# AnamarijaKic/bioinfo1

Hardware: AMD Instinct MI355X
Metric: GCUPS (DP cell updates/s) at 1/2/4/8 GPUs; bit-exact score+CIGAR (higher is better)
Workload: dtype int32 semantics; packed int16 arithmetic where range-proven (fits_int16), else int32; 1 GPU; config 2: 10000 uniform 1000x1000 pairs per GPU, local, scoring 1,-1,-1, CIGAR on; pairs_per_gpu=10000, qlen=1000, tlen=1000, mode=local, cigar=True, cells_per_gpu=10000000000, cells_total=10000000000, parallelism=pairs range-split over 1 GPU(s)

## Files before the change

bioinfo1_amd/align.py:

```python
from __future__ import annotations

import ctypes as C
import enum
import os
from dataclasses import dataclass

import numpy as np

HERE = os.path.dirname(os.path.abspath(__file__))
LIB_PATH = os.path.join(HERE, "libteam_alignment.so")

TA_OK, TA_ERR_BAD_TYPE, TA_ERR_CIGAR, TA_ERR_ARG, TA_ERR_DEVICE, TA_ERR_CAPACITY, TA_ERR_RANGE, TA_ERR_UNSERVED = range(8)
TA_PLAN_INT32_ONLY, TA_PLAN_NO_FLEX, TA_PLAN_UNFUSED, TA_PLAN_WALK1, TA_PLAN_WALK2 = 1, 2, 4, 8, 16
TA_PLAN_SERIAL_PASSES, TA_PLAN_PASS_MAJOR, TA_PLAN_NO_BLK, TA_PLAN_NO_CK, TA_PLAN_CK = 32, 64, 128, 256, 512
TA_PLAN_NO_FLEX_CK = 1024


class AlignmentType(enum.IntEnum):

    global_ = 0
    local = 1
    semiGlobal = 2


# ... 27 lines not shown
    L.ta_cigar_slot_bytes.argtypes = [C.c_uint32, C.c_uint32]
    L.ta_align_batch.argtypes = [C.c_void_p, C.c_uint32, C.c_void_p, u64p, u32p, C.c_void_p, u64p, u32p, C.c_int,
                                 C.c_int, C.c_int, C.c_int, C.c_int, i32p, u32p, C.c_void_p, C.c_uint64, u64p, u32p]
    L.ta_align_batch_flags.argtypes = L.ta_align_batch.argtypes + [C.c_uint32]
    L.ta_context_release.argtypes = [C.c_void_p]
    L.ta_context_release.restype = None
    L.ta_context_held_bytes.argtypes = [C.c_void_p]
    L.ta_context_held_bytes.restype = C.c_uint64
    L.ta_set_default_device.argtypes = [C.c_int]
    L.ta_set_thread_device.argtypes = [C.c_int]
    L.ta_plan_create.argtypes = [C.c_void_p, C.c_uint32, u32p, u32p, C.c_int, C.c_int, C.c_int, C.c_int, C.c_int,
                                 C.c_uint64, C.c_uint32, C.POINTER(C.c_void_p)]
    L.ta_plan_destroy.argtypes = [C.c_void_p]
    L.ta_plan_destroy.restype = None
    for f in ("ta_plan_cigar_slots_bytes", "ta_plan_workspace_bytes"):
        getattr(L, f).restype = C.c_uint64
        getattr(L, f).argtypes = [C.c_void_p]
    L.ta_plan_chunks.restype = C.c_uint32
    L.ta_plan_chunks.argtypes = [C.c_void_p]
    L.ta_plan_dual_pairs.restype = C.c_uint32
    L.ta_plan_dual_pairs.argtypes = [C.c_void_p]
    L.ta_plan_flex_pairs.restype = C.c_uint32
    L.ta_plan_flex_pairs.argtypes = [C.c_void_p]
    L.ta_plan_fused.argtypes = [C.c_void_p]
    L.ta_plan_walk.argtypes = [C.c_void_p]
    L.ta_plan_pair_chunks.argtypes = [C.c_void_p, u32p]
    L.ta_affine_plan_pair_chunks.argtypes = [C.c_void_p, u32p]
    L.ta_plan_execute.argtypes = [C.c_void_p, C.c_void_p, C.c_void_p]
    L.ta_plan_check.argtypes = [C.c_void_p]
    L.ta_compact_cigars.argtypes = [C.c_void_p, C.c_uint32, C.c_void_p, C.c_void_p, C.c_void_p, C.c_void_p,
                                    C.c_void_p, C.c_void_p]
    L.ta_plan_execute_fill.argtypes = [C.c_void_p, C.c_void_p, C.c_void_p, C.c_uint32]
    L.ta_plan_execute_traceback.argtypes = [C.c_void_p, C.c_void_p, C.c_void_p, C.c_uint32]
    L.ta_align_batch_affine.argtypes = [C.c_void_p, C.c_uint32, C.c_void_p, u64p, u32p, C.c_void_p, u64p, u32p,
                                        C.c_int, C.c_int, C.c_int, C.c_int, C.c_int, C.c_int, i32p, u32p, C.c_void_p,
                                        C.c_uint64, u64p, u32p]
    L.ta_affine_plan_create.argtypes = [C.c_void_p, C.c_uint32, u32p, u32p, C.c_int, C.c_int, C.c_int, C.c_int,
                                        C.c_int, C.c_int, C.c_uint64, C.c_uint32, C.POINTER(C.c_void_p)]
    L.ta_affine_plan_destroy.argtypes = [C.c_void_p]
    L.ta_affine_plan_destroy.restype = None
    for f in ("ta_affine_plan_cigar_slots_bytes", "ta_affine_plan_workspace_bytes"):
        getattr(L, f).restype = C.c_uint64
        getattr(L, f).argtypes = [C.c_void_p]
    L.ta_affine_plan_chunks.restype = C.c_uint32
    L.ta_affine_plan_chunks.argtypes = [C.c_void_p]
    L.ta_affine_plan_dual_pairs.restype = C.c_uint32
    L.ta_affine_plan_dual_pairs.argtypes = [C.c_void_p]
    L.ta_affine_plan_execute.argtypes = [C.c_void_p, C.c_void_p, C.c_void_p]
    L.ta_affine_plan_execute_fill.argtypes = [C.c_void_p, C.c_void_p, C.c_void_p, C.c_uint32]
    L.ta_affine_plan_execute_traceback.argtypes = [C.c_void_p, C.c_void_p, C.c_void_p, C.c_uint32]
    L.ta_affine_plan_check.argtypes = [C.c_void_p]
    L.ta_align_batch_banded.argtypes = [C.c_void_p, C.c_uint32, C.c_void_p, u64p, u32p, C.c_void_p, u64p, u32p, u32p,
                                        C.c_int, C.c_int, C.c_int, C.c_int, C.c_int, i32p, u32p, C.c_void_p,
                                        C.c_uint64, u64p, u32p]
    L.ta_banded_plan_create.argtypes = [C.c_void_p, C.c_uint32, u32p, u32p, u32p, C.c_int, C.c_int, C.c_int, C.c_int,
                                        C.c_int, C.c_uint64, C.c_uint32, C.POINTER(C.c_void_p)]
    L.ta_banded_plan_destroy.argtypes = [C.c_void_p]
    L.ta_banded_plan_destroy.restype = None
    for f in ("ta_banded_plan_cigar_slots_bytes", "ta_banded_plan_workspace_bytes", "ta_banded_plan_band_cells",
              "ta_banded_plan_swept_cells"):
        getattr(L, f).restype = C.c_uint64
        getattr(L, f).argtypes = [C.c_void_p]
    L.ta_banded_plan_chunks.restype = C.c_uint32
    L.ta_banded_plan_chunks.argtypes = [C.c_void_p]
    L.ta_banded_plan_pair_chunks.argtypes = [C.c_void_p, u32p]
    L.ta_banded_plan_execute.argtypes = [C.c_void_p, C.c_void_p, C.c_void_p]
    L.ta_banded_plan_execute_fill.argtypes = [C.c_void_p, C.c_void_p, C.c_void_p, C.c_uint32]
    L.ta_banded_plan_execute_traceback.argtypes = [C.c_void_p, C.c_void_p, C.c_void_p, C.c_uint32]
    L.ta_banded_plan_check.argtypes = [C.c_void_p]
    L.ta_banded_plan_annotate.argtypes = [C.c_void_p, C.c_void_p, C.c_void_p, C.c_void_p]
    L.ta_plan_annotate.argtypes = [C.c_void_p, C.c_void_p, C.c_void_p, C.c_void_p]
    L.ta_affine_plan_annotate.argtypes = [C.c_void_p, C.c_void_p, C.c_void_p, C.c_void_p]
    L.ta_server_create.argtypes = [C.c_int, C.c_int, C.c_uint32, C.POINTER(C.c_void_p)]
    L.ta_server_destroy.argtypes = [C.c_void_p]
    L.ta_server_destroy.restype = None
    L.ta_server_fits.argtypes = [C.c_void_p, C.c_uint32, C.c_uint32, C.c_int, C.c_int, C.c_int]
    L.ta_server_running.argtypes = [C.c_void_p]
    L.ta_server_last_times.argtypes = [C.c_void_p, C.c_uint32, C.POINTER(C.c_double)]
    L.ta_server_align.argtypes = [C.c_void_p, C.c_char_p, C.c_uint32, C.c_char_p, C.c_uint32, C.c_int, C.c_int,
                                  C.c_int, C.c_int, C.POINTER(C.c_int32), C.POINTER(C.c_uint32), C.c_void_p,
                                  C.c_uint64, C.POINTER(C.c_uint32)]
    _lib = L
    return L


ABI_SYMBOLS = [
    "ta_status_string", "ta_last_error", "ta_context_create", "ta_context_destroy", "ta_context_release",
    "ta_context_held_bytes", "ta_set_default_device", "ta_set_thread_device", "ta_current_device", "ta_device_count",
    "ta_cigar_slot_bytes", "ta_align_batch", "ta_align_batch_flags", "ta_plan_create", "ta_plan_destroy", "ta_plan_cigar_slots_bytes",
    "ta_plan_workspace_bytes", "ta_plan_chunks", "ta_plan_dual_pairs", "ta_plan_flex_pairs", "ta_plan_fused", "ta_plan_walk",
    "ta_plan_execute", "ta_plan_check", "ta_plan_execute_fill", "ta_plan_pair_chunks", "ta_affine_plan_pair_chunks", "ta_plan_execute_traceback", "ta_compact_cigars",
    "ta_affine_plan_create", "ta_affine_plan_destroy", "ta_affine_plan_cigar_slots_bytes",
    "ta_affine_plan_workspace_bytes", "ta_affine_plan_chunks", "ta_affine_plan_dual_pairs", "ta_affine_plan_execute", "ta_affine_plan_execute_fill",
    "ta_affine_plan_execute_traceback", "ta_affine_plan_check", "ta_align_batch_affine",
    "ta_server_create", "ta_server_destroy", "ta_server_fits", "ta_server_align", "ta_server_running",
    "ta_server_last_times", "ta_server_pause", "ta_server_resume",
    "ta_plan_annotate", "ta_affine_plan_annotate",
]
BANDED_ABI_SYMBOLS = [
    "ta_banded_plan_create", "ta_banded_plan_destroy", "ta_banded_plan_cigar_slots_bytes",
    "ta_banded_plan_workspace_bytes", "ta_banded_plan_chunks", "ta_banded_plan_pair_chunks",
    "ta_banded_plan_band_cells", "ta_banded_plan_swept_cells", "ta_banded_plan_execute",
    "ta_banded_plan_execute_fill", "ta_banded_plan_execute_traceback", "ta_banded_plan_check",
    "ta_banded_plan_annotate", "ta_align_batch_banded",
]
ABI_SYMBOLS += BANDED_ABI_SYMBOLS
TEAM_ALIGN_SYMBOL = ("_ZN4team5AlignEPKcjS1_jNS_13AlignmentTypeEiiiPNSt7__cxx1112basic_stringIcSt11char_traitsIcESaIcEEEPj")


def _check_type(type) -> int:
    t = int(type)
    if t not in (0, 1, 2):
        raise ValueError("Unknown AlignmentType provided.")
    return t


def _raise(status: int, ctx=None):
    L = lib()
    msg = L.ta_status_string(status).decode()
    if status in (TA_ERR_BAD_TYPE, TA_ERR_CIGAR, TA_ERR_RANGE):
        raise ValueError(msg)
    detail = L.ta_last_error(ctx).decode() if ctx else ""
    raise DeviceError(f"{msg}: {detail}" if detail else msg)


def _p(a, ct):
    return a.ctypes.data_as(C.POINTER(ct))


def _band_array(band, n_pairs: int) -> np.ndarray:
# ... 415 lines not shown
        idx = torch.as_tensor(np.asarray(indices, np.int64), device=self.dev)
        sc = self.score[idx].cpu().numpy()
        tb = self.target_begin[idx].cpu().numpy().view(np.uint32)
        if not self.want_cigar:
            return BatchResult(sc, tb, None, None, None)
        start = self.cigar_start[idx].cpu().numpy()
        ln = self.cigar_len[idx].cpu().numpy().view(np.uint32)
        parts, offs, o = [], np.zeros(len(ln), np.uint64), 0
        for k in range(len(ln)):
            parts.append(self.slots[int(start[k]):int(start[k]) + int(ln[k])].cpu().numpy())
            offs[k] = o
            o += int(ln[k])
        arena = np.concatenate(parts) if parts else np.zeros(1, np.uint8)
        return BatchResult(sc, tb, offs, ln, arena)

    def results(self) -> BatchResult:
        self.check()
        return _results(self)

    def close(self):
        if getattr(self, "_h", None):
            self._fn("ta_plan_destroy")(self._h)
            self._h = None

    def __del__(self):
        try:
            self.close()
        except Exception:
            pass


class DevicePipeline:

    def __init__(self, device: int, batch, type, match, mismatch, gap, want_cigar=True, depth: int = 2,
                 workspace_budget: int = 0, gap_open=None, flags: int = 0, inputs=None, first=None):
        import torch

        self.torch = torch
        self.dev = torch.device("cuda", device)
        self.aligners, self.plans = [], []
        for k in range(depth):
            if k == 0 and first is not None:
                self.plans.append(first)
                continue
            al = Aligner(device)
            self.aligners.append(al)
            shared = inputs if not self.plans else (self.plans[0].qbytes, self.plans[0].qoff,
                                                    self.plans[0].tbytes, self.plans[0].toff)
            self.plans.append(DevicePlan(al, batch, type, match, mismatch, gap, want_cigar,
                                         workspace_budget=workspace_budget, gap_open=gap_open, flags=flags,
                                         inputs=shared))
        self.fill = torch.cuda.Stream(self.dev)
        self.walk = torch.cuda.Stream(self.dev, priority=-1)
        for st in (self.fill, self.walk):
            st.wait_stream(torch.cuda.current_stream(self.dev))
        self.walked = [torch.cuda.Event() for _ in range(depth)]
        self.done = [torch.cuda.Event() for _ in range(depth)]
        self.used = [False] * depth
        self.k = 0
        self.last = None

    @property
    def chunks(self):
        return self.plans[0].chunks

    def step(self, inputs=None, ready=None):
        torch = self.torch
        cur = torch.cuda.current_stream(self.dev)
        depth = len(self.plans)
        if self.last is not None:
            self.done[self.last].record(cur)
        i = self.k % depth
        self.k += 1
        plan = self.plans[i]
        if self.used[i]:
            self.fill.wait_event(self.done[i])
        if inputs is not None:
            plan.set_inputs(inputs)
            if ready is not None:
                self.fill.wait_event(ready)
        for c in range(plan.chunks):
            with torch.cuda.stream(self.fill):
                plan.run_fill(c)
            with torch.cuda.stream(self.walk):
                plan.run_traceback(c)
        self.walked[i].record(self.walk)
        cur.wait_event(self.walked[i])
        self.used[i] = True
        self.last = i
        return plan

    def check(self):
        for p in self.plans:
            p.check()

    def close(self):
        for p in self.plans:
            p.close()
        for al in self.aligners:
            al.close()


class HostBatchRunner:

    def __init__(self, aligner: Aligner, batch, type, match, mismatch, gap, want_cigar=True):
        import torch

        self.t = _check_type(type)
        self.sc = (match, mismatch, gap)
        self.want_cigar = bool(want_cigar)
        self.aligner = aligner
        self.P = P = batch.n_pairs

        def pinned(a):
            a = np.ascontiguousarray(a)
            t = torch.empty(max(a.nbytes, 1), dtype=torch.uint8, pin_memory=True)
            v = t.numpy()[: a.nbytes].view(a.dtype)
            v[...] = a.reshape(-1)
            return t, v

        self._keep = []
        for name, a in (("qb", batch.qbytes if batch.qbytes.size else np.zeros(1, np.uint8)), ("qoff", batch.qoff),
                        ("qlen", batch.qlen), ("tb", batch.tbytes if batch.tbytes.size else np.zeros(1, np.uint8)),
                        ("toff", batch.toff), ("tlen", batch.tlen), ("score", np.zeros(P, np.int32)),
                        ("tbeg", np.zeros(P, np.uint32)), ("coff", np.zeros(P, np.uint64)),
                        ("clen", np.zeros(P, np.uint32))):
            t, v = pinned(a)
            self._keep.append(t)
            setattr(self, name, v)
# ... 130 lines not shown
```

bioinfo1_amd/csrc/ta_affine.hip:

```cpp
#include <hip/hip_runtime.h>
#include <rocprofiler-sdk-roctx/roctx.h>

#include <algorithm>
#include <cstdlib>
#include <cstring>
#include <numeric>
#include <string>
#include <vector>

#include "../../include/team_align_c.h"
#include "ta_context.h"
#include "ta_device.h"
#include "ta_host_batch.h"
#include "ta_planner.h"
#include "ta_packed.h"

namespace ta {
namespace {

constexpr int kNeg = -(1 << 29);

struct AffArgs {
    const uint32_t* order;
    uint32_t begin, count;
// ... 1222 lines not shown
    AffOffs o = aff_layout(pl->h, L);
    const uint64_t upload = L.bytes;
    aff_layout_scratch(pl->h, L, o);
    std::vector<uint8_t> host(upload);
    aff_pack(pl->h, o, host.data());
    hipError_t e = hipMalloc(&pl->own_block, std::max<uint64_t>(L.bytes, 256));
    if (e == hipSuccess) e = hipMemcpy(pl->own_block, host.data(), upload, hipMemcpyHostToDevice);
    if (e != hipSuccess) {
        ta_affine_plan_destroy(pl);
        return fail(ctx, TA_ERR_DEVICE, std::string("ta_affine_plan_create: ") + hipGetErrorString(e));
    }
    aff_bind(pl, static_cast<uint8_t*>(pl->own_block), o);
    *out = pl;
    return TA_OK;
}

uint64_t ta_affine_plan_cigar_slots_bytes(const ta_affine_plan* pl) { return pl ? pl->h.slots_bytes : 0; }

int ta_affine_plan_check(ta_affine_plan* pl) {
    if (!pl) return TA_ERR_ARG;
    if (pl->h.duals.empty() && pl->h.single_tasks.empty()) return TA_OK;
    uint32_t err = 0;
    TA_HIP(pl->ctx, hipSetDevice(pl->ctx->device));
    TA_HIP(pl->ctx, hipMemcpy(&err, pl->d_err, 4, hipMemcpyDeviceToHost));
    if (!err) return TA_OK;
    TA_HIP(pl->ctx, hipMemset(pl->d_err, 0, 4));
    return fail(pl->ctx, TA_ERR_DEVICE,
                "affine fill: a pass hand-off poll timed out; results of this plan are invalid");
}
uint64_t ta_affine_plan_workspace_bytes(const ta_affine_plan* pl) {
    return pl ? pl->h.ws_ptr_entries * sizeof(uint2) + pl->h.ws_bnd_entries * sizeof(int2) : 0;
}
uint32_t ta_affine_plan_chunks(const ta_affine_plan* pl) { return pl ? (uint32_t)pl->h.chunks.size() : 0; }
uint32_t ta_affine_plan_dual_pairs(const ta_affine_plan* pl) { return pl ? (uint32_t)pl->h.duals.size() : 0; }

int ta_affine_plan_pair_chunks(const ta_affine_plan* pl, uint32_t* chunk_of_pair) {
    if (!pl || !chunk_of_pair) return TA_ERR_ARG;
    for (uint32_t c = 0; c < (uint32_t)pl->h.chunks.size(); ++c) {
        const auto& ch = pl->h.chunks[c];
        for (uint32_t k = ch.begin; k < ch.begin + ch.count; ++k) chunk_of_pair[pl->h.order[k]] = c;
    }
    return TA_OK;
}

int ta_affine_plan_execute(ta_affine_plan* pl, const ta_device_io* io, void* stream) {
    if (int r = affine_check_io(pl, io)) return r;
    std::lock_guard<std::mutex> lock(pl->ctx->mu);
    return affine_exec(pl, io, (hipStream_t)stream, UINT32_MAX, true, true);
}

int ta_affine_plan_annotate(ta_affine_plan* pl, const ta_device_io* io, const ta_annotate_io* out, void* stream) {
    if (!pl || !io || !out) return TA_ERR_ARG;
    ta_context* ctx = pl->ctx;
    if (!pl->h.want_cigar) return fail(ctx, TA_ERR_ARG, "annotate: the plan has no CIGARs");
    if (out->eqx_slots && (!out->eqx_start || !out->eqx_len)) return fail(ctx, TA_ERR_ARG, "annotate: eqx_slots without eqx_start / eqx_len");
    if (int r = affine_check_io(pl, io)) return r;
    if (!pl->h.n_pairs) return TA_OK;
    std::lock_guard<std::mutex> lock(ctx->mu);
    TA_HIP(ctx, hipSetDevice(ctx->device));
    ta::AnnotateArgs a{pl->h.n_pairs, pl->h.type, pl->d_qlen, pl->d_tlen, pl->d_goal_i, pl->d_goal_j, pl->d_slot_off,
                       reinterpret_cast<const uint8_t*>(io->query_bytes), io->query_off,
                       reinterpret_cast<const uint8_t*>(io->target_bytes), io->target_off, io->cigar_slots,
                       io->cigar_start, io->cigar_len, out->info, out->eqx_slots, out->eqx_start, out->eqx_len};
    TA_HIP(ctx, ta::launch_annotate(a, (hipStream_t)stream));
    return TA_OK;
}
// ... 40 lines not shown
```

bioinfo1_amd/csrc/ta_api.hip:

```cpp
#include <hip/hip_runtime.h>
#include <rocprofiler-sdk-roctx/roctx.h>

#include <algorithm>
#include <cstdio>
#include <cstdlib>
#include <cstring>
#include <mutex>
#include <string>
#include <vector>

#include "../../include/team_align_c.h"
#include "ta_context.h"
#include "ta_host_batch.h"
#include "ta_internal.h"
#include "ta_planner.h"

using ta_host::fail;

struct ta_plan {
    ta_context* ctx = nullptr;
    ta::Plan h;
    void* own_block = nullptr;
    uint32_t *d_qlen = nullptr, *d_tlen = nullptr, *d_order = nullptr, *d_singles = nullptr, *d_duals = nullptr,
             *d_flexes = nullptr;
    uint64_t *d_ptr_off = nullptr, *d_bnd_off = nullptr, *d_slot_off = nullptr;
    uint32_t *d_goal_i = nullptr, *d_goal_j = nullptr;
    uint32_t* d_fb = nullptr;
    uint32_t *d_flex_task_off = nullptr, *d_tickets = nullptr, *d_err = nullptr, *d_flex_tasks = nullptr;
    void* d_pout = nullptr;
    void* d_dpout = nullptr;
    uint32_t* d_stask_off = nullptr;
    uint64_t* d_stasks = nullptr;
    void* d_spout = nullptr;
    uint8_t* d_pflag = nullptr;
};

namespace {

bool valid_type(int t) { return t == TA_GLOBAL || t == TA_LOCAL || t == TA_SEMI_GLOBAL; }

struct PlanOffs {
    uint64_t qlen, tlen, order, singles, duals, flexes, task_off, tasks, stask_off, stasks, ptr_off, bnd_off, slot_off,
        err, tickets;
    uint64_t goal_i, goal_j, fb, pout, dpout, spout, pflag;
};

uint64_t dual_pout_bytes(const ta::Plan& h) {
// ... 182 lines not shown
                if (ch.fcount) {
                    if (int r = ta_host::lazy_stream(ctx, ctx->aux2)) return r;
                    TA_HIP(ctx, hipEventRecord(ctx->ev_fork, s));
                    TA_HIP(ctx, hipStreamWaitEvent(ctx->aux2, ctx->ev_fork, 0));
                    TA_HIP(ctx, ta::launch_dual(h.type, h.want_cigar, d, ctx->aux2));
                    TA_HIP(ctx, hipEventRecord(ctx->ev_join2, ctx->aux2));
                } else {
                    TA_HIP(ctx, ta::launch_dual(h.type, h.want_cigar, d, s));
                }
            }
            if (ch.fcount) {
                ta::FillArgs d = a;
                d.order = pl->d_flexes;
                d.begin = ch.fbegin;
                d.count = ch.fcount;
                d.fb_list = fb_list;
                d.fb_count = fb_count;
                d.task_off = pl->d_flex_task_off;
                d.tasks = pl->d_flex_tasks;
                d.ticket = pl->d_tickets + c;
                d.n_tasks = h.flex_task_off[ch.fbegin + ch.fcount] - h.flex_task_off[ch.fbegin];
                d.epoch = ++ctx->epoch & 0x3FFFFFFu;
                d.err = pl->d_err;
                d.pout = pl->d_pout;
                TA_HIP(ctx, hipMemsetAsync(d.ticket, 0, 4, s));
                TA_HIP(ctx, ta::launch_flex(h.type, h.want_cigar, d, s));
            }
            if (ch.dcount && ch.fcount) TA_HIP(ctx, hipStreamWaitEvent(s, ctx->ev_join2, 0));
            ta::FillArgs f = a;
            f.order = fb_list;
            f.begin = 0;
            f.count = 2 * (ch.dcount + ch.fcount);
            f.count_dev = fb_count;
            TA_HIP(ctx, ta::launch_fill(h.type, h.want_cigar, h.wide, f, s));
        }
        if (ch.scount && (ch.dcount || ch.fcount)) {
            TA_HIP(ctx, hipEventRecord(ctx->ev_join, ctx->aux));
            TA_HIP(ctx, hipStreamWaitEvent(s, ctx->ev_join, 0));
        }
        roctxRangePop();
    }
    if (trace && h.want_cigar && !h.fused) {
        roctxRangePushA("ta traceback");
        ta::TraceArgs t{};
        t.order = pl->d_order;
        t.begin = ch.begin;
        t.count = ch.count;
        t.qlen = pl->d_qlen;
        t.tlen = pl->d_tlen;
        t.ptrs = d_ptrs;
        t.ptr_off = pl->d_ptr_off;
        t.goal_i = pl->d_goal_i;
        t.goal_j = pl->d_goal_j;
        t.slots = io->cigar_slots;
        t.slot_off = pl->d_slot_off;
        t.cigar_start = io->cigar_start;
        t.cigar_len = io->cigar_len;
        t.score = io->score;
        t.qbytes = reinterpret_cast<const uint8_t*>(io->query_bytes);
        t.qoff = io->query_off;
        t.tbytes = reinterpret_cast<const uint8_t*>(io->target_bytes);
        t.toff = io->target_off;
        t.match = h.match;
        t.mismatch = h.mismatch;
        t.gap = h.gap;
        t.blk = h.blk ? (h.ck ? 2u : 1u) : 0u;
// ... 147 lines not shown
    if (!out) return TA_ERR_ARG;
    *out = nullptr;
    if (int r = check_args(ctx, n_pairs, qlen, tlen, type)) return r;
    TA_HIP(ctx, hipSetDevice(ctx->device));
    auto* pl = new ta_plan();
    pl->ctx = ctx;
    ta::build_plan(pl->h, n_pairs, qlen, tlen, type, match, mismatch, gap, want_cigar != 0,
                   budget ? budget : ta_host::default_budget(ctx), flags, 4 * ctx->cu_count);
    ta::BlockLayout L;
    PlanOffs o = layout_uploaded(pl->h, L);
    const uint64_t upload = L.bytes;
    layout_scratch(pl->h, L, o);
    std::vector<uint8_t> host(upload);
    pack(pl->h, o, host.data());
    hipError_t e = hipMalloc(&pl->own_block, std::max<uint64_t>(L.bytes, 256));
    if (e == hipSuccess) e = hipMemcpy(pl->own_block, host.data(), upload, hipMemcpyHostToDevice);
    if (e != hipSuccess) {
        ta_plan_destroy(pl);
        return fail(ctx, TA_ERR_DEVICE, std::string("ta_plan_create: ") + hipGetErrorString(e));
    }
    bind(pl, static_cast<uint8_t*>(pl->own_block), o);
    *out = pl;
    return TA_OK;
}

uint64_t ta_plan_cigar_slots_bytes(const ta_plan* pl) { return pl ? pl->h.slots_bytes : 0; }
uint64_t ta_plan_workspace_bytes(const ta_plan* pl) {
    if (!pl) return 0;
    const ta::Plan& h = pl->h;
    const uint64_t runs = (h.walk_group == 64 && h.want_cigar) ? 4 * (h.slots_bytes + 4) : 0;
    return (h.ws_ptr_dwords + h.ws_bnd_words) * 4ull + runs;
}
uint32_t ta_plan_chunks(const ta_plan* pl) { return pl ? (uint32_t)pl->h.chunks.size() : 0; }
uint32_t ta_plan_dual_pairs(const ta_plan* pl) { return pl ? pl->h.n_dual_pairs : 0; }
uint32_t ta_plan_flex_pairs(const ta_plan* pl) { return pl ? (uint32_t)pl->h.flexes.size() : 0; }
int ta_plan_fused(const ta_plan* pl) { return pl && pl->h.fused ? 1 : 0; }

int ta_plan_walk(const ta_plan* pl) {
    if (!pl) return -1;
    return pl->h.walk_group | (pl->h.blk ? 0x100 : 0) | (pl->h.ck ? 0x200 : 0);
}

int ta_plan_pair_chunks(const ta_plan* pl, uint32_t* chunk_of_pair) {
    if (!pl || !chunk_of_pair) return TA_ERR_ARG;
    for (uint32_t c = 0; c < (uint32_t)pl->h.chunks.size(); ++c) {
        const auto& ch = pl->h.chunks[c];
        for (uint32_t k = ch.begin; k < ch.begin + ch.count; ++k) chunk_of_pair[pl->h.order[k]] = c;
    }
    return TA_OK;
}

int ta_plan_execute(ta_plan* pl, const ta_device_io* io, void* stream) {
    if (int r = check_io(pl, io)) return r;
    std::lock_guard<std::mutex> lock(pl->ctx->mu);
    return exec(pl, io, (hipStream_t)stream, UINT32_MAX, true, true);
}

int ta_plan_execute_fill(ta_plan* pl, const ta_device_io* io, void* stream, uint32_t chunk) {
    if (int r = check_io(pl, io)) return r;
    if (chunk >= pl->h.chunks.size()) return pl->h.n_pairs ? TA_ERR_ARG : TA_OK;
    std::lock_guard<std::mutex> lock(pl->ctx->mu);
    return exec(pl, io, (hipStream_t)stream, chunk, true, false);
}

int ta_plan_execute_traceback(ta_plan* pl, const ta_device_io* io, void* stream, uint32_t chunk) {
    if (int r = check_io(pl, io)) return r;
// ... 75 lines not shown
```

bioinfo1_amd/csrc/ta_internal.h:

```cpp
#pragma once

#include <hip/hip_runtime.h>
#include <stdint.h>

#include "../../include/team_align_c.h"
#include "ta_layout.h"

namespace ta {

enum Code : uint32_t { kCodeM = 0, kCodeI = 1, kCodeD = 2, kCodeStop = 3 };
constexpr int kDPlane = 16;

struct FillArgs {
    const uint32_t* order;
    uint32_t begin, count;
    const uint8_t* qbytes;
    const uint64_t* qoff;
    const uint32_t* qlen;
    const uint8_t* tbytes;
    const uint64_t* toff;
    const uint32_t* tlen;
    int match, mismatch, gap;
    uint32_t* ptrs;
    const uint64_t* ptr_off;
    int32_t* bnd;
    const uint64_t* bnd_off;
    int32_t* score;
    uint32_t* target_begin;
    uint32_t* goal_i;
    uint32_t* goal_j;
    int fused;
    char* slots;
    const uint64_t* slot_off;
    uint64_t* cigar_start;
    uint32_t* cigar_len;
    uint32_t* fb_list;
    uint32_t* fb_count;
    const uint32_t* count_dev;
    const uint32_t* task_off;
    const uint32_t* tasks;
    uint32_t* ticket;
    uint32_t n_tasks;
    uint32_t epoch;
    uint32_t* err;
    void* pout;
    const uint64_t* tasks64;
    uint32_t end_aligned;
    uint32_t blk;
    uint8_t* pflag;
};

constexpr uint32_t kErrPassPoll = 1u;
constexpr uint32_t kErrWalkCap = 2u;
__host__ __device__ inline uint64_t band_runs_off(uint64_t slot_off) { return (slot_off + 3u) & ~(uint64_t)3u; }

struct TraceArgs {
    const uint32_t* order;
    uint32_t begin, count;
    const uint32_t* qlen;
    const uint32_t* tlen;
    const uint32_t* ptrs;
    const uint64_t* ptr_off;
    const uint32_t* goal_i;
    const uint32_t* goal_j;
    char* slots;
    const uint64_t* slot_off;
    uint64_t* cigar_start;
    uint32_t* cigar_len;
    const int32_t* score;
    const uint8_t* qbytes;
    const uint64_t* qoff;
// ... 97 lines not shown
```

bioinfo1_amd/csrc/ta_kernels.hip:

```cpp
#include <algorithm>
#include <cstdlib>

#include "ta_device.h"
#include "ta_walk2.h"
#include "ta_walk_lane.h"
#include "ta_walk_band.h"

namespace ta {
namespace {

#ifdef TA_FILL_MODE
struct PairOut {
    int score;
    uint32_t tb, gi, gj;
    uint64_t cstart;
    uint32_t clen;
};

template <int MODE>
__device__ __forceinline__ PairOut degenerate(int gap, uint32_t n, uint32_t m) {
    PairOut o{0, 0, 0, 0, 0, 0};
    if (MODE == kGlobal) {
        o.gi = n;
        o.gj = m;
// ... 319 lines not shown
        const WalkSeq seq{Q, T, best_h, a.match, a.mismatch, a.gap};
        traceback_pair<MODE>(ptrs, n, m, o.gi, o.gj, slot, cigar_slot_bytes(n, m), lane, &o.cstart, &o.clen, seq);
    }
    return o;
}

template <int MODE, bool CIGAR, bool WIDE>
__device__ __forceinline__ void fill_pair(const FillArgs& a, uint32_t p, int lane) {
    const uint32_t n = a.qlen[p], m = a.tlen[p];
    const bool walk = CIGAR && a.fused;
    uint32_t* ptrs = (CIGAR && n && m) ? a.ptrs + a.ptr_off[p] : nullptr;
    int32_t* B = (n_passes(n) > 1) ? a.bnd + a.bnd_off[p] : nullptr;
    char* slot = walk ? a.slots + a.slot_off[p] : nullptr;
    const PairOut o = fill_one<MODE, CIGAR, WIDE>(a, n, m, a.qbytes + a.qoff[p], a.tbytes + a.toff[p], ptrs, B, slot,
                                                  walk, lane);
    if (lane == 0) {
        a.score[p] = o.score;
        a.target_begin[p] = o.tb;
        a.goal_i[p] = o.gi;
        a.goal_j[p] = o.gj;
        if (walk) {
            a.cigar_start[p] = a.slot_off[p] + o.cstart;
            a.cigar_len[p] = o.clen;
        }
    }
}

template <int MODE, bool CIGAR, bool WIDE>
__global__ __launch_bounds__(kBlock) void fill_kernel(FillArgs a) {
    const int lane = threadIdx.x & 63;
    const uint32_t widx = wave_id();
    if (widx >= (a.count_dev ? *a.count_dev : a.count)) return;
    fill_pair<MODE, CIGAR, WIDE>(a, a.order ? a.order[a.begin + widx] : a.begin + widx, lane);
}

template <int MODE, bool CIGAR, bool WIDE>
__global__ __launch_bounds__(kBlock) void fill_pipe_kernel(FillArgs a) {
    const int lane = threadIdx.x & 63;
    uint32_t tk = 0;
    if (lane == 0) tk = atomicAdd(a.ticket, 1u);
    tk = (uint32_t)__builtin_amdgcn_readfirstlane((int)tk);
    if (tk >= a.n_tasks) return;
    const uint64_t code = a.tasks64[a.task_off[a.begin] + tk];
    const uint32_t w = (uint32_t)(code >> 32), pass = (uint32_t)code;
    const uint32_t p = a.order[w];
    const uint32_t n = a.qlen[p], m = a.tlen[p];
    const bool last_pass = pass + 1 == n_passes(n);
    uint64_t* rec = reinterpret_cast<uint64_t*>(a.bnd + a.bnd_off[p]);
    const uint64_t rb = (uint64_t)m + 1;
    const BndIo B{nullptr, last_pass ? nullptr : rec + (pass & 1u) * rb, pass ? rec + ((pass - 1u) & 1u) * rb : nullptr,
                  pass + 1u, pass, a.err};
    uint32_t* ptrs = CIGAR ? a.ptrs + a.ptr_off[p] : nullptr;
    const PassOut o = run_pass_any<MODE, CIGAR, WIDE>(a, a.qbytes + a.qoff[p], a.tbytes + a.toff[p], n, m, pass,
                                                      last_pass, ptrs, B, lane);
    if (lane == 0) static_cast<PassOut*>(a.pout)[a.task_off[w] + pass] = o;
}

template <int MODE>
__global__ void fill_combine_kernel(FillArgs a) {
    const uint32_t w = a.begin + blockIdx.x * blockDim.x + threadIdx.x;
    if (w >= a.begin + a.count) return;
    const uint32_t p = a.order[w];
    const uint32_t n = a.qlen[p], m = a.tlen[p];
    PairOut r;
    if (n == 0 || m == 0) {
        r = degenerate<MODE>(a.gap, n, m);
// ... 406 lines not shown
        }
    }
}

__global__ __launch_bounds__(kBlock) void format_runs_kernel(TraceArgs a) {
    const uint32_t w = wave_id();
    if (w >= a.count) return;
    format_runs(a, a.order ? a.order[a.begin + w] : a.begin + w, threadIdx.x & 63);
}

__global__ __launch_bounds__(kBlock) void compact_kernel(CompactArgs a) {
    const int lane = threadIdx.x & 63;
    const uint32_t p = wave_id();
    if (p >= a.n_pairs) return;
    const char* src = a.slots + a.cigar_start[p];
    char* dst = a.dst + a.dst_off[p];
    const uint32_t len = a.cigar_len[p];
    for (uint32_t k = (uint32_t)lane; k < len; k += 64u) dst[k] = src[k];
}

#endif

inline dim3 grid_for(uint32_t waves) { return dim3((waves + kWavesPerBlock - 1) / kWavesPerBlock); }

}

#ifdef TA_FILL_MODE
template <>
hipError_t launch_fill_mode<TA_FILL_MODE, (TA_FILL_CIGAR != 0)>(bool wide, const FillArgs& a, hipStream_t s) {
    constexpr int MODE = TA_FILL_MODE;
    constexpr bool CIGAR = TA_FILL_CIGAR != 0;
    if (!a.count) return hipSuccess;
    const dim3 g = grid_for(a.count), b(kBlock);
    if (a.tasks64) {
        if (a.n_tasks) {
            const dim3 gt = grid_for(a.n_tasks);
            if (MODE == kLocal && wide) hipLaunchKernelGGL((fill_pipe_kernel<MODE, CIGAR, MODE == kLocal>), gt, b, 0, s, a);
            else hipLaunchKernelGGL((fill_pipe_kernel<MODE, CIGAR, false>), gt, b, 0, s, a);
        }
        hipLaunchKernelGGL(fill_combine_kernel<MODE>, dim3((a.count + 255) / 256), dim3(256), 0, s, a);
        return hipGetLastError();
    }
    if (MODE == kLocal && wide) hipLaunchKernelGGL((fill_kernel<MODE, CIGAR, MODE == kLocal>), g, b, 0, s, a);
    else hipLaunchKernelGGL((fill_kernel<MODE, CIGAR, false>), g, b, 0, s, a);
    return hipGetLastError();
}
#if TA_FILL_CIGAR
template <>
hipError_t launch_serve_mode<TA_FILL_MODE>(const ServeArgs& a, uint32_t slots, hipStream_t s) {
    hipLaunchKernelGGL(serve_kernel<TA_FILL_MODE>, dim3(slots), dim3(kWave), 0, s, a);
    return hipGetLastError();
}
#endif
#endif

#ifdef TA_TU_MISC
#ifndef TA_LW_G
#define TA_LW_G 16
#endif
hipError_t launch_fill(int mode, bool cigar, bool wide, const FillArgs& a, hipStream_t s) {
    switch (mode * 2 + (cigar ? 1 : 0)) {
        case 0: return launch_fill_mode<kGlobal, false>(wide, a, s);
        case 1: return launch_fill_mode<kGlobal, true>(wide, a, s);
        case 2: return launch_fill_mode<kLocal, false>(wide, a, s);
        case 3: return launch_fill_mode<kLocal, true>(wide, a, s);
        case 4: return launch_fill_mode<kSemi, false>(wide, a, s);
// ... 101 lines not shown
```

include/team_align_c.h:

```cpp
#ifndef TEAM_ALIGN_C_H
#define TEAM_ALIGN_C_H

#include <stddef.h>
#include <stdint.h>

#ifdef __cplusplus
extern "C" {
#endif

#define TA_GLOBAL 0
#define TA_LOCAL 1
#define TA_SEMI_GLOBAL 2

#define TA_OK 0
#define TA_ERR_BAD_TYPE 1
#define TA_ERR_CIGAR 2
#define TA_ERR_ARG 3
#define TA_ERR_DEVICE 4
#define TA_ERR_CAPACITY 5

typedef struct ta_context ta_context;
typedef struct ta_plan ta_plan;

const char* ta_status_string(int status);
// ... 50 lines not shown
#define TA_PLAN_NO_FLEX_CK 1024u
int ta_plan_create(ta_context* ctx, uint32_t n_pairs, const uint32_t* query_len_host,
                   const uint32_t* target_len_host, int type, int match, int mismatch, int gap, int want_cigar,
                   uint64_t workspace_budget, uint32_t flags, ta_plan** out);
void ta_plan_destroy(ta_plan* plan);
uint64_t ta_plan_cigar_slots_bytes(const ta_plan* plan);
uint64_t ta_plan_workspace_bytes(const ta_plan* plan);
uint32_t ta_plan_chunks(const ta_plan* plan);
uint32_t ta_plan_dual_pairs(const ta_plan* plan);
uint32_t ta_plan_flex_pairs(const ta_plan* plan);
int ta_plan_fused(const ta_plan* plan);
int ta_plan_walk(const ta_plan* plan);
int ta_plan_pair_chunks(const ta_plan* plan, uint32_t* chunk_of_pair);

typedef struct ta_device_io {
    const char* query_bytes;
    const uint64_t* query_off;
    const char* target_bytes;
    const uint64_t* target_off;
    int32_t* score;
    uint32_t* target_begin;
    char* cigar_slots;
    uint64_t* cigar_start;
    uint32_t* cigar_len;
} ta_device_io;

int ta_plan_execute(ta_plan* plan, const ta_device_io* io, void* hip_stream);

int ta_plan_check(ta_plan* plan);

int ta_plan_execute_fill(ta_plan* plan, const ta_device_io* io, void* hip_stream, uint32_t chunk);
int ta_plan_execute_traceback(ta_plan* plan, const ta_device_io* io, void* hip_stream, uint32_t chunk);

int ta_compact_cigars(ta_context* ctx, uint32_t n_pairs, const char* cigar_slots, const uint64_t* cigar_start,
                      const uint32_t* cigar_len, const uint64_t* dst_off, char* dst, void* hip_stream);

typedef struct ta_pair_info {
    uint32_t query_begin, query_end;
    uint32_t target_begin, target_end;
    uint32_t n_eq, n_x, n_ins, n_del;
    uint32_t n_gap_runs;
    uint32_t n_free;
} ta_pair_info;

typedef struct ta_annotate_io {
    ta_pair_info* info;
    char* eqx_slots;
    uint64_t* eqx_start;
    uint32_t* eqx_len;
} ta_annotate_io;

int ta_plan_annotate(ta_plan* plan, const ta_device_io* io, const ta_annotate_io* out, void* hip_stream);

#define TA_ERR_RANGE 6
#define TA_ERR_UNSERVED 7

typedef struct ta_affine_plan ta_affine_plan;

int ta_affine_plan_create(ta_context* ctx, uint32_t n_pairs, const uint32_t* query_len_host,
                          const uint32_t* target_len_host, int type, int match, int mismatch, int gap_open,
                          int gap_extend, int want_cigar, uint64_t workspace_budget, uint32_t flags,
                          ta_affine_plan** out);
void ta_affine_plan_destroy(ta_affine_plan* plan);
uint64_t ta_affine_plan_cigar_slots_bytes(const ta_affine_plan* plan);
uint64_t ta_affine_plan_workspace_bytes(const ta_affine_plan* plan);
uint32_t ta_affine_plan_chunks(const ta_affine_plan* plan);
uint32_t ta_affine_plan_dual_pairs(const ta_affine_plan* plan);
int ta_affine_plan_pair_chunks(const ta_affine_plan* plan, uint32_t* chunk_of_pair);
int ta_affine_plan_execute(ta_affine_plan* plan, const ta_device_io* io, void* hip_stream);
int ta_affine_plan_execute_fill(ta_affine_plan* plan, const ta_device_io* io, void* hip_stream, uint32_t chunk);
int ta_affine_plan_execute_traceback(ta_affine_plan* plan, const ta_device_io* io, void* hip_stream,
                                     uint32_t chunk);
int ta_affine_plan_check(ta_affine_plan* plan);
int ta_affine_plan_annotate(ta_affine_plan* plan, const ta_device_io* io, const ta_annotate_io* out,
                            void* hip_stream);

int ta_align_batch_affine(ta_context* ctx, uint32_t n_pairs, const char* query_bytes, const uint64_t* query_off,
                          const uint32_t* query_len, const char* target_bytes, const uint64_t* target_off,
                          const uint32_t* target_len, int type, int match, int mismatch, int gap_open,
                          int gap_extend, int want_cigar, int32_t* score, uint32_t* target_begin,
                          char* cigar_arena, uint64_t cigar_arena_bytes, uint64_t* cigar_off, uint32_t* cigar_len);

typedef struct ta_banded_plan ta_banded_plan;

int ta_banded_plan_create(ta_context* ctx, uint32_t n_pairs, const uint32_t* query_len_host,
                          const uint32_t* target_len_host, const uint32_t* band_host, int type, int match,
                          int mismatch, int gap, int want_cigar, uint64_t workspace_budget, uint32_t flags,
                          ta_banded_plan** out);
void ta_banded_plan_destroy(ta_banded_plan* plan);
uint64_t ta_banded_plan_cigar_slots_bytes(const ta_banded_plan* plan);
uint64_t ta_banded_plan_workspace_bytes(const ta_banded_plan* plan);
uint32_t ta_banded_plan_chunks(const ta_banded_plan* plan);
int ta_banded_plan_pair_chunks(const ta_banded_plan* plan, uint32_t* chunk_of_pair);
uint64_t ta_banded_plan_band_cells(const ta_banded_plan* plan);
uint64_t ta_banded_plan_swept_cells(const ta_banded_plan* plan);
int ta_banded_plan_execute(ta_banded_plan* plan, const ta_device_io* io, void* hip_stream);
int ta_banded_plan_execute_fill(ta_banded_plan* plan, const ta_device_io* io, void* hip_stream, uint32_t chunk);
int ta_banded_plan_execute_traceback(ta_banded_plan* plan, const ta_device_io* io, void* hip_stream,
                                     uint32_t chunk);
int ta_banded_plan_check(ta_banded_plan* plan);
int ta_banded_plan_annotate(ta_banded_plan* plan, const ta_device_io* io, const ta_annotate_io* out,
                            void* hip_stream);

int ta_align_batch_banded(ta_context* ctx, uint32_t n_pairs, const char* query_bytes, const uint64_t* query_off,
                          const uint32_t* query_len, const char* target_bytes, const uint64_t* target_off,
                          const uint32_t* target_len, const uint32_t* band, int type, int match, int mismatch,
// ... 9 lines not shown
```

Measured before the change: 7358 GCUPS.

## Move multi-slot fill/traceback pipeline into native code with per-slot fill streams

Replaces the Python/torch stream-and-event pipeline with a native ta_pipeline that gives each slot its own fill stream and shares one high-priority traceback stream. It also raises the default pipeline depth from 2 to 3 and adds a persistent grid-stride fallback fill kernel, capped at the CU count, for device-counted work. The aim is to cut Python launch overhead and let fills of consecutive batches overlap. The costs are one more set of workspace buffers and more complex cross-stream dependencies.

```diff
diff --git a/bioinfo1_amd/align.py b/bioinfo1_amd/align.py
--- a/bioinfo1_amd/align.py
+++ b/bioinfo1_amd/align.py
@@ -83,6 +83,11 @@
                                     C.c_void_p, C.c_void_p]
     L.ta_plan_execute_fill.argtypes = [C.c_void_p, C.c_void_p, C.c_void_p, C.c_uint32]
     L.ta_plan_execute_traceback.argtypes = [C.c_void_p, C.c_void_p, C.c_void_p, C.c_uint32]
+    L.ta_pipeline_create.argtypes = [C.POINTER(C.c_void_p), C.c_uint32, C.POINTER(C.c_void_p)]
+    L.ta_pipeline_create_affine.argtypes = L.ta_pipeline_create.argtypes
+    L.ta_pipeline_step.argtypes = [C.c_void_p, C.c_void_p, C.c_void_p, C.c_void_p, u32p]
+    L.ta_pipeline_destroy.argtypes = [C.c_void_p]
+    L.ta_pipeline_destroy.restype = None
     L.ta_align_batch_affine.argtypes = [C.c_void_p, C.c_uint32, C.c_void_p, u64p, u32p, C.c_void_p, u64p, u32p,
                                         C.c_int, C.c_int, C.c_int, C.c_int, C.c_int, C.c_int, i32p, u32p, C.c_void_p,
                                         C.c_uint64, u64p, u32p]
@@ -147,6 +152,8 @@
     "ta_server_create", "ta_server_destroy", "ta_server_fits", "ta_server_align", "ta_server_running",
     "ta_server_last_times", "ta_server_pause", "ta_server_resume",
     "ta_plan_annotate", "ta_affine_plan_annotate",
+    "ta_plan_context", "ta_affine_plan_context", "ta_context_device",
+    "ta_pipeline_create", "ta_pipeline_create_affine", "ta_pipeline_step", "ta_pipeline_destroy",
 ]
 BANDED_ABI_SYMBOLS = [
     "ta_banded_plan_create", "ta_banded_plan_destroy", "ta_banded_plan_cigar_slots_bytes",
@@ -628,13 +635,13 @@
 
 class DevicePipeline:
 
-    def __init__(self, device: int, batch, type, match, mismatch, gap, want_cigar=True, depth: int = 2,
+    def __init__(self, device: int, batch, type, match, mismatch, gap, want_cigar=True, depth: int = 3,
                  workspace_budget: int = 0, gap_open=None, flags: int = 0, inputs=None, first=None):
         import torch
 
         self.torch = torch
         self.dev = torch.device("cuda", device)
-        self.aligners, self.plans = [], []
+        self.aligners, self.plans, self.k = [], [], 0
         for k in range(depth):
             if k == 0 and first is not None:
                 self.plans.append(first)
@@ -646,44 +653,40 @@
             self.plans.append(DevicePlan(al, batch, type, match, mismatch, gap, want_cigar,
                                          workspace_budget=workspace_budget, gap_open=gap_open, flags=flags,
                                          inputs=shared))
-        self.fill = torch.cuda.Stream(self.dev)
-        self.walk = torch.cuda.Stream(self.dev, priority=-1)
-        for st in (self.fill, self.walk):
-            st.wait_stream(torch.cuda.current_stream(self.dev))
-        self.walked = [torch.cuda.Event() for _ in range(depth)]
-        self.done = [torch.cuda.Event() for _ in range(depth)]
-        self.used = [False] * depth
-        self.k = 0
-        self.last = None
+        L = lib()
+        handles = (C.c_void_p * len(self.plans))(*[p._h for p in self.plans])
+        h = C.c_void_p()
+        create = L.ta_pipeline_create_affine if self.plans[0].affine else L.ta_pipeline_create
+        r = create(handles, len(self.plans), C.byref(h))
+        if r != TA_OK:
+            msg = L.ta_last_error(self.plans[0]._ctx).decode()
+            for p in self.plans[1 if first is not None else 0:]:
+                p.close()
+            for al in self.aligners:
+                al.close()
+            if r == TA_ERR_ARG:
+                raise ValueError(msg or "ta_pipeline_create: invalid argument")
+            raise DeviceError(f"{L.ta_status_string(r).decode()}: {msg}")
+        self._h = h
 
     @property
     def chunks(self):
         return self.plans[0].chunks
 
     def step(self, inputs=None, ready=None):
-        torch = self.torch
-        cur = torch.cuda.current_stream(self.dev)
-        depth = len(self.plans)
-        if self.last is not None:
-            self.done[self.last].record(cur)
-        i = self.k % depth
-        self.k += 1
-        plan = self.plans[i]
-        if self.used[i]:
-            self.fill.wait_event(self.done[i])
+        if ready is not None and inputs is None:
+            raise ValueError("DevicePipeline.step: ready without inputs (the event belongs to an upload of inputs)")
+        plan = self.plans[self.k % len(self.plans)]
         if inputs is not None:
             plan.set_inputs(inputs)
-            if ready is not None:
-                self.fill.wait_event(ready)
-        for c in range(plan.chunks):
-            with torch.cuda.stream(self.fill):
-                plan.run_fill(c)
-            with torch.cuda.stream(self.walk):
-                plan.run_traceback(c)
-        self.walked[i].record(self.walk)
-        cur.wait_event(self.walked[i])
-        self.used[i] = True
-        self.last = i
+        cur = self.torch.cuda.current_stream(self.dev)
+        slot = C.c_uint32()
+        ev = C.c_void_p(ready.cuda_event) if ready is not None else None
+        r = lib().ta_pipeline_step(self._h, C.byref(plan.io), ev, C.c_void_p(cur.cuda_stream), C.byref(slot))
+        if r != TA_OK:
+            _raise(r, plan._ctx)
+        assert self.plans[slot.value] is plan
+        self.k += 1
         return plan
 
     def check(self):
@@ -691,6 +694,9 @@
             p.check()
 
     def close(self):
+        if getattr(self, "_h", None):
+            lib().ta_pipeline_destroy(self._h)
+            self._h = None
         for p in self.plans:
             p.close()
         for al in self.aligners:
diff --git a/bioinfo1_amd/csrc/ta_affine.hip b/bioinfo1_amd/csrc/ta_affine.hip
--- a/bioinfo1_amd/csrc/ta_affine.hip
+++ b/bioinfo1_amd/csrc/ta_affine.hip
@@ -1278,6 +1278,7 @@
     return pl ? pl->h.ws_ptr_entries * sizeof(uint2) + pl->h.ws_bnd_entries * sizeof(int2) : 0;
 }
 uint32_t ta_affine_plan_chunks(const ta_affine_plan* pl) { return pl ? (uint32_t)pl->h.chunks.size() : 0; }
+ta_context* ta_affine_plan_context(const ta_affine_plan* pl) { return pl ? pl->ctx : nullptr; }
 uint32_t ta_affine_plan_dual_pairs(const ta_affine_plan* pl) { return pl ? (uint32_t)pl->h.duals.size() : 0; }
 
 int ta_affine_plan_pair_chunks(const ta_affine_plan* pl, uint32_t* chunk_of_pair) {
diff --git a/bioinfo1_amd/csrc/ta_api.hip b/bioinfo1_amd/csrc/ta_api.hip
--- a/bioinfo1_amd/csrc/ta_api.hip
+++ b/bioinfo1_amd/csrc/ta_api.hip
@@ -13,6 +13,7 @@
 #include "ta_context.h"
 #include "ta_host_batch.h"
 #include "ta_internal.h"
+#include "ta_pipeline_internal.h"
 #include "ta_planner.h"
 
 using ta_host::fail;
@@ -261,6 +262,7 @@
             f.begin = 0;
             f.count = 2 * (ch.dcount + ch.fcount);
             f.count_dev = fb_count;
+            f.max_blocks = ctx->cu_count;
             TA_HIP(ctx, ta::launch_fill(h.type, h.want_cigar, h.wide, f, s));
         }
         if (ch.scount && (ch.dcount || ch.fcount)) {
@@ -474,6 +476,11 @@
     return (h.ws_ptr_dwords + h.ws_bnd_words) * 4ull + runs;
 }
 uint32_t ta_plan_chunks(const ta_plan* pl) { return pl ? (uint32_t)pl->h.chunks.size() : 0; }
+ta_context* ta_plan_context(const ta_plan* pl) { return pl ? pl->ctx : nullptr; }
+int ta_context_device(const ta_context* ctx) { return ctx ? ctx->device : -1; }
+void ta_context_set_error(ta_context* ctx, const char* message) {
+    if (ctx) ctx->last_error = message ? message : "";
+}
 uint32_t ta_plan_dual_pairs(const ta_plan* pl) { return pl ? pl->h.n_dual_pairs : 0; }
 uint32_t ta_plan_flex_pairs(const ta_plan* pl) { return pl ? (uint32_t)pl->h.flexes.size() : 0; }
 int ta_plan_fused(const ta_plan* pl) { return pl && pl->h.fused ? 1 : 0; }
diff --git a/bioinfo1_amd/csrc/ta_internal.h b/bioinfo1_amd/csrc/ta_internal.h
--- a/bioinfo1_amd/csrc/ta_internal.h
+++ b/bioinfo1_amd/csrc/ta_internal.h
@@ -37,6 +37,7 @@
     uint32_t* fb_list;
     uint32_t* fb_count;
     const uint32_t* count_dev;
+    uint32_t max_blocks;
     const uint32_t* task_off;
     const uint32_t* tasks;
     uint32_t* ticket;
diff --git a/bioinfo1_amd/csrc/ta_kernels.hip b/bioinfo1_amd/csrc/ta_kernels.hip
--- a/bioinfo1_amd/csrc/ta_kernels.hip
+++ b/bioinfo1_amd/csrc/ta_kernels.hip
@@ -375,6 +375,15 @@
     const uint32_t widx = wave_id();
     if (widx >= (a.count_dev ? *a.count_dev : a.count)) return;
     fill_pair<MODE, CIGAR, WIDE>(a, a.order ? a.order[a.begin + widx] : a.begin + widx, lane);
+}
+
+template <int MODE, bool CIGAR, bool WIDE>
+__global__ __launch_bounds__(kBlock) void fill_back_kernel(FillArgs a) {
+    const int lane = threadIdx.x & 63;
+    const uint32_t count = *a.count_dev;
+    const uint32_t stride = gridDim.x * kWavesPerBlock;
+    for (uint32_t widx = wave_id(); widx < count; widx += stride)
+        fill_pair<MODE, CIGAR, WIDE>(a, a.order[a.begin + widx], lane);
 }
 
 template <int MODE, bool CIGAR, bool WIDE>
@@ -847,6 +856,12 @@
     constexpr bool CIGAR = TA_FILL_CIGAR != 0;
     if (!a.count) return hipSuccess;
     const dim3 g = grid_for(a.count), b(kBlock);
+    if (a.count_dev && a.max_blocks) {
+        const dim3 gb(std::min<uint32_t>(g.x, a.max_blocks));
+        if (MODE == kLocal && wide) hipLaunchKernelGGL((fill_back_kernel<MODE, CIGAR, MODE == kLocal>), gb, b, 0, s, a);
+        else hipLaunchKernelGGL((fill_back_kernel<MODE, CIGAR, false>), gb, b, 0, s, a);
+        return hipGetLastError();
+    }
     if (a.tasks64) {
         if (a.n_tasks) {
             const dim3 gt = grid_for(a.n_tasks);
diff --git a/bioinfo1_amd/csrc/ta_pipeline.cpp b/bioinfo1_amd/csrc/ta_pipeline.cpp
--- /dev/null
+++ b/bioinfo1_amd/csrc/ta_pipeline.cpp
@@ -0,0 +1,185 @@
+#ifndef __HIP_PLATFORM_AMD__
+#define __HIP_PLATFORM_AMD__ 1
+#endif
+#include <hip/hip_runtime_api.h>
+
+#include <string>
+#include <vector>
+
+#include "../../include/team_align_c.h"
+#include "ta_pipeline_internal.h"
+
+namespace {
+
+struct Ops {
+    ta_context* (*context)(const void*);
+    uint32_t (*chunks)(const void*);
+    int (*fill)(void*, const ta_device_io*, void*, uint32_t);
+    int (*walk)(void*, const ta_device_io*, void*, uint32_t);
+};
+
+const Ops kLinear = {
+    [](const void* p) { return ta_plan_context(static_cast<const ta_plan*>(p)); },
+    [](const void* p) { return ta_plan_chunks(static_cast<const ta_plan*>(p)); },
+    [](void* p, const ta_device_io* io, void* s, uint32_t c) {
+        return ta_plan_execute_fill(static_cast<ta_plan*>(p), io, s, c);
+    },
+    [](void* p, const ta_device_io* io, void* s, uint32_t c) {
+        return ta_plan_execute_traceback(static_cast<ta_plan*>(p), io, s, c);
+    },
+};
+
+const Ops kAffine = {
+    [](const void* p) { return ta_affine_plan_context(static_cast<const ta_affine_plan*>(p)); },
+    [](const void* p) { return ta_affine_plan_chunks(static_cast<const ta_affine_plan*>(p)); },
+    [](void* p, const ta_device_io* io, void* s, uint32_t c) {
+        return ta_affine_plan_execute_fill(static_cast<ta_affine_plan*>(p), io, s, c);
+    },
+    [](void* p, const ta_device_io* io, void* s, uint32_t c) {
+        return ta_affine_plan_execute_traceback(static_cast<ta_affine_plan*>(p), io, s, c);
+    },
+};
+
+int fail(ta_context* ctx, int code, const std::string& msg) {
+    ta_context_set_error(ctx, msg.c_str());
+    return code;
+}
+
+#define TP_HIP(ctx, expr)                                                                     \
+    do {                                                                                      \
+        hipError_t e_ = (expr);                                                               \
+        if (e_ != hipSuccess)                                                                 \
+            return fail((ctx), TA_ERR_DEVICE, std::string(#expr) + ": " + hipGetErrorString(e_)); \
+    } while (0)
+
+}
+
+struct ta_pipeline {
+    const Ops* ops = nullptr;
+    int device = 0;
+    std::vector<void*> slots;
+    std::vector<ta_context*> ctxs;
+    std::vector<hipStream_t> fill;
+    hipStream_t walk = nullptr;
+    std::vector<hipEvent_t> done, walked;
+    hipEvent_t start = nullptr;
+    std::vector<bool> used;
+    uint64_t k = 0;
+    int last = -1;
+};
+
+namespace {
+
+int create(const Ops& ops, void* const* slots, uint32_t depth, ta_pipeline** out) {
+    if (!out) return TA_ERR_ARG;
+    *out = nullptr;
+    if (!slots || !depth || !slots[0]) return TA_ERR_ARG;
+    ta_context* c0 = ops.context(slots[0]);
+    if (!c0) return TA_ERR_ARG;
+    if (depth < 2) return fail(c0, TA_ERR_ARG, "ta_pipeline_create: depth must be at least 2");
+    for (uint32_t a = 0; a < depth; ++a) {
+        ta_context* ca = slots[a] ? ops.context(slots[a]) : nullptr;
+        if (!ca) return fail(c0, TA_ERR_ARG, "ta_pipeline_create: null slot");
+        if (ta_context_device(ca) != ta_context_device(c0))
+            return fail(c0, TA_ERR_ARG, "ta_pipeline_create: slots on different devices");
+        for (uint32_t b = 0; b < a; ++b)
+            if (ops.context(slots[b]) == ca)
+                return fail(c0, TA_ERR_ARG, "ta_pipeline_create: two slots share a context (each needs its own workspace)");
+    }
+    auto* p = new ta_pipeline();
+    p->ops = &ops;
+    p->device = ta_context_device(c0);
+    p->slots.assign(slots, slots + depth);
+    for (uint32_t a = 0; a < depth; ++a) p->ctxs.push_back(ops.context(slots[a]));
+    p->fill.assign(depth, nullptr);
+    p->done.assign(depth, nullptr);
+    p->walked.assign(depth, nullptr);
+    p->used.assign(depth, false);
+    *out = p;
+    return TA_OK;
+}
+
+int lazy_stream(ta_context* ctx, hipStream_t& s, int priority) {
+    if (s) return TA_OK;
+    if (hipStreamCreateWithPriority(&s, hipStreamNonBlocking, priority) != hipSuccess) {
+        s = nullptr;
+        return fail(ctx, TA_ERR_DEVICE, "ta_pipeline_step: hipStreamCreateWithPriority failed");
+    }
+    return TA_OK;
+}
+
+int lazy_event(ta_context* ctx, hipEvent_t& e) {
+    if (e) return TA_OK;
+    if (hipEventCreateWithFlags(&e, hipEventDisableTiming) != hipSuccess) {
+        e = nullptr;
+        return fail(ctx, TA_ERR_DEVICE, "ta_pipeline_step: hipEventCreateWithFlags failed");
+    }
+    return TA_OK;
+}
+
+}
+
+extern "C" {
+
+int ta_pipeline_create(ta_plan* const* slots, uint32_t depth, ta_pipeline** out) {
+    return create(kLinear, reinterpret_cast<void* const*>(slots), depth, out);
+}
+
+int ta_pipeline_create_affine(ta_affine_plan* const* slots, uint32_t depth, ta_pipeline** out) {
+    return create(kAffine, reinterpret_cast<void* const*>(slots), depth, out);
+}
+
+int ta_pipeline_step(ta_pipeline* p, const ta_device_io* io, void* ready_event, void* caller_stream,
+                     uint32_t* slot_out) {
+    if (!p) return TA_ERR_ARG;
+    const uint32_t depth = (uint32_t)p->slots.size();
+    const uint32_t i = (uint32_t)(p->k % depth);
+    ta_context* ctx = p->ctxs[i];
+    if (!io) return fail(ctx, TA_ERR_ARG, "ta_pipeline_step: null io");
+    hipStream_t cur = static_cast<hipStream_t>(caller_stream);
+    TP_HIP(ctx, hipSetDevice(p->device));
+    if (!p->walk) {
+        int least = 0, greatest = 0;
+        TP_HIP(ctx, hipDeviceGetStreamPriorityRange(&least, &greatest));
+        if (int r = lazy_stream(ctx, p->walk, greatest)) return r;
+    }
+    if (int r = lazy_stream(ctx, p->fill[i], 0)) return r;
+    if (int r = lazy_event(ctx, p->done[i])) return r;
+    if (int r = lazy_event(ctx, p->walked[i])) return r;
+    if (!p->start) {
+        if (int r = lazy_event(ctx, p->start)) return r;
+        TP_HIP(ctx, hipEventRecord(p->start, cur));
+    }
+    if (p->last >= 0) TP_HIP(ctx, hipEventRecord(p->done[p->last], cur));
+    if (slot_out) *slot_out = i;
+    void* plan = p->slots[i];
+    TP_HIP(ctx, hipStreamWaitEvent(p->fill[i], p->used[i] ? p->done[i] : p->start, 0));
+    if (ready_event) TP_HIP(ctx, hipStreamWaitEvent(p->fill[i], static_cast<hipEvent_t>(ready_event), 0));
+    const uint32_t chunks = p->ops->chunks(plan);
+    for (uint32_t c = 0; c < chunks; ++c) {
+        if (int r = p->ops->fill(plan, io, p->fill[i], c)) return r;
+        if (int r = p->ops->walk(plan, io, p->walk, c)) return r;
+    }
+    TP_HIP(ctx, hipEventRecord(p->walked[i], p->walk));
+    TP_HIP(ctx, hipStreamWaitEvent(cur, p->walked[i], 0));
+    p->used[i] = true;
+    p->last = (int)i;
+    ++p->k;
+    return TA_OK;
+}
+
+void ta_pipeline_destroy(ta_pipeline* p) {
+    if (!p) return;
+    (void)hipSetDevice(p->device);
+    for (hipStream_t s : p->fill)
+        if (s) (void)hipStreamDestroy(s);
+    if (p->walk) (void)hipStreamDestroy(p->walk);
+    for (hipEvent_t e : p->done)
+        if (e) (void)hipEventDestroy(e);
+    for (hipEvent_t e : p->walked)
+        if (e) (void)hipEventDestroy(e);
+    if (p->start) (void)hipEventDestroy(p->start);
+    delete p;
+}
+
+}
diff --git a/bioinfo1_amd/csrc/ta_pipeline_internal.h b/bioinfo1_amd/csrc/ta_pipeline_internal.h
--- /dev/null
+++ b/bioinfo1_amd/csrc/ta_pipeline_internal.h
@@ -0,0 +1,13 @@
+#pragma once
+
+#include "../../include/team_align_c.h"
+
+#ifdef __cplusplus
+extern "C" {
+#endif
+
+void ta_context_set_error(ta_context* ctx, const char* message);
+
+#ifdef __cplusplus
+}
+#endif
diff --git a/include/team_align_c.h b/include/team_align_c.h
--- a/include/team_align_c.h
+++ b/include/team_align_c.h
@@ -106,6 +106,15 @@
 int ta_plan_execute_fill(ta_plan* plan, const ta_device_io* io, void* hip_stream, uint32_t chunk);
 int ta_plan_execute_traceback(ta_plan* plan, const ta_device_io* io, void* hip_stream, uint32_t chunk);
 
+ta_context* ta_plan_context(const ta_plan* plan);
+int ta_context_device(const ta_context* ctx);
+
+typedef struct ta_pipeline ta_pipeline;
+int ta_pipeline_create(ta_plan* const* slots, uint32_t depth, ta_pipeline** out);
+int ta_pipeline_step(ta_pipeline* pipe, const ta_device_io* io, void* ready_event, void* caller_stream,
+                     uint32_t* slot_out);
+void ta_pipeline_destroy(ta_pipeline* pipe);
+
 int ta_compact_cigars(ta_context* ctx, uint32_t n_pairs, const char* cigar_slots, const uint64_t* cigar_start,
                       const uint32_t* cigar_len, const uint64_t* dst_off, char* dst, void* hip_stream);
 
@@ -146,6 +155,8 @@
 int ta_affine_plan_execute_traceback(ta_affine_plan* plan, const ta_device_io* io, void* hip_stream,
                                      uint32_t chunk);
 int ta_affine_plan_check(ta_affine_plan* plan);
+ta_context* ta_affine_plan_context(const ta_affine_plan* plan);
+int ta_pipeline_create_affine(ta_affine_plan* const* slots, uint32_t depth, ta_pipeline** out);
 int ta_affine_plan_annotate(ta_affine_plan* plan, const ta_device_io* io, const ta_annotate_io* out,
                             void* hip_stream);
 
```

Result: faster. 7948 GCUPS, median of 6 (+8.0%).
